# skhu101/HumanLiff

Measured on AMD Instinct MI355X. Metric: denoise-steps/sec, higher is better.
Workload: dtype f32; 1 GPU; configs[1]: 256x256x27 tri-plane UNet (controlnet, 497M params), 1000-step DDPM p_sample_loop, batch=4 per GPU; global_batch=4, parallelism=replicas x1 (subjects sharded, final all-gather only)

## Files before the change

humanliff_amd/csrc/hl_unet.cpp:

```cpp
#include <cstdint>
#include <string>
#include <unordered_map>
#include <utility>
#include <vector>

#include "hl_unet_kernels.h"
#include <algorithm>

namespace {

using hl::ConvArgs;
using hl::View;

static inline int round_up(int v, int m) { return (v + m - 1) / m * m; }

bool conv_mode_known(int mode) {
    return mode == HL_CONV_FP32 || mode == HL_CONV_FP32_MFMA || mode == HL_CONV_BF16X3 || mode == HL_CONV_FP32_DIRECT || mode == HL_CONV_FP32_F23 ||
           mode == HL_CONV_BF16 || mode == HL_CONV_FP16;
}
struct ConvForms { bool bf3, wino, wino4, h2, h16; };
ConvForms conv_forms(int mode, bool bf16_h16, bool bwd_data) {
    const bool f32 = mode == HL_CONV_FP32 || mode == HL_CONV_FP32_MFMA || mode == HL_CONV_FP16;
    ConvForms f;
    f.bf3 = mode == HL_CONV_BF16X3 || mode == HL_CONV_BF16;
    f.wino = f32 || mode == HL_CONV_FP32_F23;
    f.wino4 = f32;
    f.h2 = mode == HL_CONV_FP32 && !bwd_data;
    f.h16 = mode == HL_CONV_FP16 || (bf16_h16 && mode == HL_CONV_BF16);
    return f;
}

struct Conv {
    const float *w = nullptr;
    const void *w_bf3 = nullptr;
    const float *w_wino = nullptr;
    const void *w_h2 = nullptr;
    const void *w_h16 = nullptr;
    const float *w_wino4 = nullptr;
    const float *bias = nullptr;
    int Cin = 0, Cin_pad = 0, Cout = 0, ks = 1;
};
struct Norm {
    const float *gamma = nullptr, *beta = nullptr;
    int C = 0;
    float eps = 1e-5f;
};
struct Res {
    Norm n1, n2;
    Conv c1, c2, skip;
    bool has_skip = false;
    bool aware = false;
    long emb_off = 0;
    int Cin = 0, Cout = 0;
};
struct Attn {
    Norm norm;
    Conv qkv, proj;
    int C = 0, heads = 1;
};
struct Xf {
    Norm norm;
    Conv proj_in, proj_out, qkv, out1, ff_in, ff_out;
    const float *ln1_g = nullptr, *ln1_b = nullptr, *ln3_g = nullptr, *ln3_b = nullptr;
    const float *v2_w = nullptr, *o2_w = nullptr, *o2_b = nullptr;
    int C = 0, heads = 1;
};
enum Kind { K_CONV, K_RES, K_ATTN, K_DOWN, K_UP, K_XF };
struct Layer {
    Kind kind;
    int idx;
};
struct Block {
    std::vector<Layer> layers;
    int Cout = 0;
    int ds_out = 1;
};

struct Net {
    hl_unet_cfg cfg{};
    std::unordered_map<std::string, std::pair<const float *, int64_t>> sd;
    std::vector<Conv> convs;
    std::vector<Res> res;
    std::vector<Attn> attn;
    std::vector<Xf> xf;
    std::vector<Block> in_blocks, out_blocks, cond_blocks;
    Block middle;
    std::vector<int> proj_cond;
    Conv out_conv;
    Norm out_norm;
    const float *te0_w = nullptr, *te0_b = nullptr, *te2_w = nullptr, *te2_b = nullptr, *label = nullptr;
    Conv ada1, ada2;
    const float *ada_w = nullptr, *ada_b = nullptr;
    const float *emb_w = nullptr, *emb_b = nullptr;
    long emb_total = 0;
    int E = 0;
    int Cpad0 = 0;
    float *packed = nullptr;
    size_t packed_off = 0;
    bool dry = true;
    hipStream_t st = nullptr;
    std::string err;
    hipStream_t side = nullptr;
    hipEvent_t ev_fork = nullptr, ev_join = nullptr;
    std::vector<hipEvent_t> ev_block;
    bool overlap = true;
    int conv_mode = 0;
    bool prof = false;
    std::vector<hipEvent_t> ev_pool;
    struct Span { int cat; size_t a, b; double flops, exec; int key[5]; long mid; };
    double dom[4] = {0, 0, 0, 0};
    int dom_key[5] = {0, 0, 0, 0, 0};
    std::vector<Span> spans;
    size_t ev_used = 0;
    int64_t census[5][8] = {};
    ~Net() {
        for (auto e : ev_pool) if (e) hipEventDestroy(e);
        for (auto e : ev_block) if (e) hipEventDestroy(e);
        if (ev_fork) hipEventDestroy(ev_fork);
        if (ev_join) hipEventDestroy(ev_join);
        if (side) hipStreamDestroy(side);
    }
    size_t next_event() {
        if (ev_used == ev_pool.size()) {
            hipEvent_t e = nullptr;
            if (hipEventCreate(&e) != hipSuccess) { if (err.empty()) err = "hipEventCreate failed (profiling events)"; e = nullptr; }
            ev_pool.push_back(e);
        }
        return ev_used++;
    }
};
enum { CAT_CONV = 0, CAT_GN = 1, CAT_ATTN = 2, CAT_OTHER = 3, CAT_N = 4 };

const float *lookup(Net &n, const std::string &name, int64_t expect) {
    if (n.dry) return reinterpret_cast<const float *>(16);
    auto it = n.sd.find(name);
    if (it == n.sd.end()) { if (n.err.empty()) n.err = "missing state_dict key: " + name; return nullptr; }
    if (expect >= 0 && it->second.second != expect) {
        if (n.err.empty()) n.err = "shape mismatch for " + name + ": got " + std::to_string(it->second.second) + " elements, expected " + std::to_string(expect);
        return nullptr;
    }
    return it->second.first;
}

Conv make_conv_w(Net &n, const float *w, const float *bias, int Cin, int Cout, int ks);
Conv make_conv(Net &n, const std::string &p, int Cin, int Cout, int ks, bool has_bias = true) {
    const float *w = lookup(n, p + ".weight", (int64_t)Cout * Cin * ks * ks);
    const float *b = has_bias ? lookup(n, p + ".bias", Cout) : nullptr;
    return make_conv_w(n, w, b, Cin, Cout, ks);
}
Conv make_conv_w(Net &n, const float *w, const float *bias, int Cin, int Cout, int ks) {
    Conv c;
    c.Cin = Cin; c.Cin_pad = round_up(Cin, 16); c.Cout = Cout; c.ks = ks;
    c.bias = n.dry ? nullptr : bias;
    const int cp = c.Cin_pad;
    size_t wino4 = hl::conv_packed_wino4_bytes(Cout, cp, ks);
    if (wino4 > ((size_t)64 << 20)) wino4 = 0;
    const size_t bytes[6] = {hl::conv_packed_floats(Cout, cp, ks) * sizeof(float), hl::conv_packed_bf3_bytes(Cout, cp, ks),
                             hl::conv_packed_wino_bytes(Cout, cp, ks), wino4, hl::conv_packed_h2_bytes(Cout, cp, ks),
                             hl::conv_packed_h16_bytes(Cout, cp, ks)};
    for (int f = 0; f < 6; ++f) {
        if (!bytes[f]) continue;
        float *dst = n.dry ? nullptr : n.packed + n.packed_off;
        n.packed_off += (bytes[f] / 4 + 63) / 64 * 64;
        if (n.dry || !w) continue;
        int rc = 0;
        switch (f) {
        case 0: rc = hl::conv_pack_weights(w, Cout, Cin, cp, ks, dst, n.st); c.w = dst; break;
        case 1: rc = hl::conv_pack_weights_bf3(w, Cout, Cin, cp, ks, dst, n.st); c.w_bf3 = dst; break;
        case 2: rc = hl::conv_pack_weights_wino(w, Cout, Cin, cp, dst, n.st); c.w_wino = dst; break;
        case 3: rc = hl::conv_pack_weights_wino4(w, Cout, Cin, cp, dst, n.st); c.w_wino4 = dst; break;
        case 4: rc = hl::conv_pack_weights_h2(w, Cout, Cin, cp, ks, dst, n.st); c.w_h2 = dst; break;
        default: rc = hl::conv_pack_weights_h16(w, Cout, Cin, cp, ks, dst, 1, n.st); c.w_h16 = dst; break;
        }
        if (rc != 0 && n.err.empty()) n.err = hl_last_error();
    }
    return c;
}
Norm make_norm(Net &n, const std::string &p, int C) {
    Norm g;
    g.C = C;
    g.gamma = lookup(n, p + ".weight", C);
    g.beta = lookup(n, p + ".bias", C);
    return g;
}

struct EmbPiece { std::string name; int O; long off; };

int add_res(Net &n, std::vector<EmbPiece> &emb, const std::string &p, int Cin, int Cout, bool aware = false) {
    Res r;
    r.Cin = Cin; r.Cout = Cout; r.aware = aware;
    r.n1 = make_norm(n, p + ".in_layers.0", Cin);
    r.c1 = make_conv(n, p + ".in_layers.2", Cin, Cout, 3);
    r.emb_off = n.emb_total;
    const int emb_o = n.cfg.no_scale_shift ? Cout : 2 * Cout;
    emb.push_back({p + ".emb_layers.1", emb_o, n.emb_total});
    n.emb_total += emb_o;
    r.n2 = make_norm(n, p + ".out_layers.0", Cout);
    r.c2 = make_conv(n, p + ".out_layers.3", aware ? 3 * Cout : Cout, Cout, 3);
    r.has_skip = Cin != Cout;
    if (r.has_skip) {
        int ks = 1;
        if (!n.dry) {
            auto it = n.sd.find(p + ".skip_connection.weight");
            if (it != n.sd.end() && it->second.second == (int64_t)Cout * Cin * 9) ks = 3;
        }
        r.skip = make_conv(n, p + ".skip_connection", Cin, Cout, ks);
        if (n.dry) n.packed_off += hl::conv_packed_floats(Cout, round_up(Cin, 16), 3) * 5;
    }
    n.res.push_back(r);
    return (int)n.res.size() - 1;
}
int add_attn(Net &n, const std::string &p, int C, int heads) {
    Attn a;
    a.C = C; a.heads = heads;
    a.norm = make_norm(n, p + ".norm", C);
    a.qkv = make_conv(n, p + ".qkv", C, 3 * C, 1);
    a.proj = make_conv(n, p + ".proj_out", C, C, 1);
    n.attn.push_back(a);
    return (int)n.attn.size() - 1;
}
int add_xf(Net &n, const std::string &p, int C, int heads) {
    Xf a;
    a.C = C; a.heads = heads;
    a.norm = make_norm(n, p + ".norm", C);
    a.norm.eps = 1e-6f;
    a.proj_in = make_conv(n, p + ".proj_in", C, C, 1);
    const std::string t = p + ".transformer_blocks.0";
    const int d = C / heads;
    const float *wq = lookup(n, t + ".attn1.to_q.weight", (int64_t)C * C), *wk = lookup(n, t + ".attn1.to_k.weight", (int64_t)C * C),
                *wv = lookup(n, t + ".attn1.to_v.weight", (int64_t)C * C);
    float *fused = n.dry ? nullptr : n.packed + n.packed_off;
    n.packed_off += ((size_t)3 * C * C + 63) / 64 * 64;
    if (!n.dry && wq && wk && wv) {
        const float *src[3] = {wq, wk, wv};
        for (int h = 0; h < heads; ++h)
            for (int q = 0; q < 3; ++q)
                hipMemcpyAsync(fused + ((size_t)h * 3 + q) * d * C, src[q] + (size_t)h * d * C, (size_t)d * C * sizeof(float), hipMemcpyDeviceToDevice, n.st);
    }
    a.qkv = make_conv_w(n, n.dry ? reinterpret_cast<const float *>(16) : fused, nullptr, C, 3 * C, 1);
    a.out1 = make_conv(n, t + ".attn1.to_out.0", C, C, 1);
    a.ln1_g = lookup(n, t + ".norm1.weight", C); a.ln1_b = lookup(n, t + ".norm1.bias", C);
    a.ln3_g = lookup(n, t + ".norm3.weight", C); a.ln3_b = lookup(n, t + ".norm3.bias", C);
    a.v2_w = lookup(n, t + ".attn2.to_v.weight", (int64_t)C * n.E);
    a.o2_w = lookup(n, t + ".attn2.to_out.0.weight", (int64_t)C * C);
    a.o2_b = lookup(n, t + ".attn2.to_out.0.bias", C);
    a.ff_in = make_conv(n, t + ".ff.net.0.proj", C, 8 * C, 1);
    a.ff_out = make_conv(n, t + ".ff.net.2", 4 * C, C, 1);
    a.proj_out = make_conv(n, p + ".proj_out", C, C, 1);
    n.xf.push_back(a);
    return (int)n.xf.size() - 1;
}
int add_conv(Net &n, const std::string &p, int Cin, int Cout, int ks) {
    n.convs.push_back(make_conv(n, p, Cin, Cout, ks));
    return (int)n.convs.size() - 1;
}
bool has_ds(const hl_unet_cfg &c, int ds) {
    for (int i = 0; i < c.n_attention_ds; ++i)
        if (c.attention_ds[i] == ds) return true;
    return false;
}

void build_encoder(Net &n, std::vector<EmbPiece> &emb, const std::string &root, std::vector<Block> &blocks,
                   std::vector<int> &chans, bool aware) {
    const hl_unet_cfg &c = n.cfg;
    Block b0;
    b0.layers.push_back({K_CONV, add_conv(n, root + ".0.0", c.in_channels, c.model_channels, 3)});
    b0.Cout = c.model_channels;
    b0.ds_out = 1;
    blocks.push_back(b0);
    chans.push_back(c.model_channels);
    int ch = c.model_channels, ds = 1, bi = 1;
    for (int level = 0; level < c.n_levels; ++level) {
        for (int r = 0; r < c.num_res_blocks; ++r) {
            Block b;
            const std::string p = root + "." + std::to_string(bi);
            const int co = c.channel_mult[level] * c.model_channels;
            b.layers.push_back({K_RES, add_res(n, emb, p + ".0", ch, co, aware)});
            ch = co;
            if (has_ds(c, ds)) {
                if (c.cross_attn) b.layers.push_back({K_XF, add_xf(n, p + ".1", ch, c.num_heads)});
                else b.layers.push_back({K_ATTN, add_attn(n, p + ".1", ch, c.num_heads)});
            }
            b.Cout = ch; b.ds_out = ds;
            blocks.push_back(b);
            chans.push_back(ch);
            ++bi;
        }
        if (level != c.n_levels - 1) {
            Block b;
            const std::string p = root + "." + std::to_string(bi);
            b.layers.push_back({K_DOWN, add_conv(n, p + ".0.op", ch, ch, 3)});
            ds *= 2;
            b.Cout = ch; b.ds_out = ds;
            blocks.push_back(b);
            chans.push_back(ch);
            ++bi;
        }
    }
}

void build(Net &n) {
    const hl_unet_cfg &c = n.cfg;
    n.E = 4 * c.model_channels;
    n.Cpad0 = round_up(c.in_channels, 16);
    n.emb_total = 0;
    n.packed_off = 0;
    n.convs.clear(); n.res.clear(); n.attn.clear(); n.xf.clear();
    n.in_blocks.clear(); n.out_blocks.clear(); n.cond_blocks.clear(); n.proj_cond.clear();
    std::vector<EmbPiece> emb;
    n.te0_w = lookup(n, "time_embed.0.weight", (int64_t)n.E * c.model_channels);
    n.te0_b = lookup(n, "time_embed.0.bias", n.E);
    n.te2_w = lookup(n, "time_embed.2.weight", (int64_t)n.E * n.E);
    n.te2_b = lookup(n, "time_embed.2.bias", n.E);
    n.label = c.num_classes > 0 ? lookup(n, "label_emb.weight", (int64_t)c.num_classes * n.E) : nullptr;
    if (c.adagn || c.cross_attn) {
        n.ada1 = make_conv(n, "conv_proj_1", c.out_channels, 6, 3);
        n.ada2 = make_conv(n, "conv_proj_2", 6, 1, 3);
        n.ada_w = lookup(n, "linear.weight", (int64_t)n.E * 4096);
        n.ada_b = lookup(n, "linear.bias", n.E);
    }

    std::vector<int> chans;
    const bool aware = c.aware3d != 0;
    build_encoder(n, emb, "input_blocks", n.in_blocks, chans, aware);
    int ch = chans.back();
    int ds = n.in_blocks.back().ds_out;
    {
        Block m;
        m.layers.push_back({K_RES, add_res(n, emb, "middle_block.0", ch, ch, aware)});
        if (c.cross_attn) m.layers.push_back({K_XF, add_xf(n, "middle_block.1", ch, c.num_heads)});
        else m.layers.push_back({K_ATTN, add_attn(n, "middle_block.1", ch, c.num_heads)});
        m.layers.push_back({K_RES, add_res(n, emb, "middle_block.2", ch, ch, aware)});
        m.Cout = ch; m.ds_out = ds;
        n.middle = m;
    }
    std::vector<int> stack = chans;
    int bi = 0;
    for (int level = c.n_levels - 1; level >= 0; --level) {
        for (int i = 0; i <= c.num_res_blocks; ++i) {
            Block b;
            const std::string p = "output_blocks." + std::to_string(bi);
            const int skip = stack.back();
            stack.pop_back();
            const int co = c.model_channels * c.channel_mult[level];
            int li = 0;
            b.layers.push_back({K_RES, add_res(n, emb, p + "." + std::to_string(li++), ch + skip, co, aware)});
            ch = co;
            if (has_ds(c, ds)) {
                if (c.cross_attn) b.layers.push_back({K_XF, add_xf(n, p + "." + std::to_string(li++), ch, c.num_heads)});
                else b.layers.push_back({K_ATTN, add_attn(n, p + "." + std::to_string(li++), ch, c.num_heads_upsample)});
            }
            if (level && i == c.num_res_blocks) {
                b.layers.push_back({K_UP, add_conv(n, p + "." + std::to_string(li++) + ".conv", ch, ch, 3)});
                ds /= 2;
            }
            b.Cout = ch; b.ds_out = ds;
            n.out_blocks.push_back(b);
            ++bi;
        }
    }
    n.out_norm = make_norm(n, "out.0", ch);
    n.out_conv = make_conv(n, "out.2", c.model_channels, c.out_channels, 3);
    if (c.controlnet) {
        std::vector<int> cch;
        build_encoder(n, emb, "input_blocks_cond", n.cond_blocks, cch, false);
        for (size_t i = 0; i < n.cond_blocks.size(); ++i)
            n.proj_cond.push_back(add_conv(n, "input_blocks_proj_cond." + std::to_string(i), cch[i], cch[i], 1));
    }
    const size_t wfl = (size_t)n.emb_total * n.E;
    if (!n.dry) {
        float *wdst = n.packed + n.packed_off, *bdst = wdst + wfl;
        for (auto &e : emb) {
            const float *w = lookup(n, e.name + ".weight", (int64_t)e.O * n.E);
            const float *b = lookup(n, e.name + ".bias", e.O);
            if (!w || !b) continue;
            hipMemcpyAsync(wdst + (size_t)e.off * n.E, w, (size_t)e.O * n.E * sizeof(float), hipMemcpyDeviceToDevice, n.st);
            hipMemcpyAsync(bdst + e.off, b, (size_t)e.O * sizeof(float), hipMemcpyDeviceToDevice, n.st);
        }
        n.emb_w = wdst; n.emb_b = bdst;
    }
    n.packed_off += (wfl + n.emb_total + 63) / 64 * 64;
}

struct Exec {
    Net &n;
    bool run;
    char *ws;
    size_t off = 0;
    hipStream_t st;
    int B, H, W;
    float *emb_all = nullptr;
    const float *ctx = nullptr;
    float *gn_scratch = nullptr;
    float *splitk_ws = nullptr;
    float *gn_scratch2 = nullptr, *splitk_ws2 = nullptr;
    float *act_ws = nullptr, *act_ws2 = nullptr;
    size_t act_need = 0;
    int rc = 0;
    struct StatReg { float *buf; int viewC, c0, covered; };
    struct PartInfo { float *buf; int viewC, c0; };
    std::unordered_map<const float *, PartInfo> part_reg;
    char *stat_base = nullptr;
    size_t stat_off = 0, stat_bytes = 0;
    float *alloc_stat(size_t floats) {
        float *p = run ? reinterpret_cast<float *>(stat_base + stat_off) : nullptr;
        stat_off += (floats * sizeof(float) + 255) / 256 * 256;
        return p;
    }
    std::unordered_map<const float *, StatReg> stat_reg;
    bool want_stats = true;

    float *alloc(size_t floats) {
        float *p = run ? reinterpret_cast<float *>(ws + off) : nullptr;
        off += (floats * sizeof(float) + 255) / 256 * 256;
        return p;
    }
    View plain(int ds, int C) {
        View v;
        v.N = B; v.H = H / ds; v.W = W / ds; v.C = C; v.pitch = C;
        v.p = alloc((size_t)v.pixels() * C);
        return v;
    }
    void ok(int r) { if (r && !rc) rc = r; }
    size_t span_begin() {
        if (!n.prof) return 0;
        const size_t a = n.next_event();
        if (n.ev_pool[a]) hipEventRecord(n.ev_pool[a], st);
        return a;
    }
    void span_end(int cat, size_t a, double flops, double exec = -1.0) {
        if (!n.prof) return;
        if (!n.err.empty() && !rc) rc = hl::fail(HL_ERR_RUNTIME, "hl_unet_forward: %s", n.err.c_str());
        const size_t b = n.next_event();
        if (n.ev_pool[b]) hipEventRecord(n.ev_pool[b], st);
        n.spans.push_back({cat, a, b, flops, exec < 0 ? flops : exec, {span_key[0], span_key[1], span_key[2], span_key[3], span_key[4]}, span_mid});
        span_key[0] = -1; span_mid = -1;
    }
    int span_key[5] = {-1, 0, 0, 0, 0};
    long span_mid = -1;

    struct Aff { float *cA = nullptr, *cB = nullptr; hl::GnSrc gn{}; bool on = false; };
    const Aff none{};
    void conv(const Conv &c, const View &in, const View &out, int stride, int ups, const Aff &af, int act,
              const float *res, long res_pitch, float *out2 = nullptr, long out2_pitch = 0, const float *res2 = nullptr,
              long res2_pitch = 0, int nchw = 0) {
        const float *cA = af.cA, *cB = af.cB;
        if (!run) {
            const size_t need = (size_t)in.pixels() * c.Cin_pad;
            if (need > act_need) act_need = need;
        }
        const bool st_ok = want_stats && !nchw;
        PartInfo pi1{nullptr, c.Cout, 0}, pi2{nullptr, c.Cout, 0};
        if (st_ok) {
            auto f1 = run ? part_reg.find(out.p) : part_reg.end();
            if (f1 != part_reg.end()) pi1 = f1->second; else pi1.buf = alloc_stat(hl::conv_stats_floats(B, (long)out.H * out.W));
            if (out2_pitch != 0) {
                auto f2 = run ? part_reg.find(out2) : part_reg.end();
                if (f2 != part_reg.end()) pi2 = f2->second; else pi2.buf = alloc_stat(hl::conv_stats_floats(B, (long)out.H * out.W));
            }
        }
        float *st1 = pi1.buf, *st2 = pi2.buf;
        if (!run) return;
        ConvArgs a{};
        a.in = in; a.in.C = c.Cin_pad;
        const ConvForms f = conv_forms(n.conv_mode, false, false);
        a.w = c.w; a.w_bf3 = f.bf3 ? c.w_bf3 : nullptr; a.bf16_single = n.conv_mode == HL_CONV_BF16;
        a.w_wino = f.wino ? c.w_wino : nullptr; a.w_wino4 = f.wino4 ? c.w_wino4 : nullptr;
        a.w_h16 = f.h16 ? c.w_h16 : nullptr; a.h16_fp16 = 1;
        a.w_h2 = f.h2 ? c.w_h2 : nullptr;
        a.bias = c.bias; a.Cout = c.Cout; a.ks = c.ks; a.stride = stride; a.ups = ups;
        a.coefA = cA; a.coefB = cB; a.act = act; a.gn = af.gn;
        a.out = out; a.res = res; a.res_pitch = res_pitch;
        a.out2 = out2; a.out2_pitch = out2_pitch; a.res2 = res2; a.res2_pitch = res2_pitch; a.out_nchw = nchw;
        a.splitk_ws = splitk_ws; a.splitk_ws_bytes = hl::conv_splitk_ws_bytes();
        a.act_ws = act_ws; a.act_ws_bytes = act_need * sizeof(float);
        a.stats = st1; a.stats2 = st2;
        if (af.cA == nullptr && af.gn.gt == nullptr) a.in_stats = raw_totals(in);
        a.st_cg = pi1.viewC / 32; a.st_c0 = pi1.c0; a.st2_cg = pi2.viewC / 32; a.st2_c0 = pi2.c0;
        const size_t e0 = span_begin();
        size_t emid = 0;
        if (n.prof) { emid = n.next_event(); a.ev_mid = n.ev_pool[emid]; }
        const hl::ConvPlan pl = hl::plan_conv(a);
        ok(hl::conv2d(a, pl, st));
        {
            static const int audit_ = [] { const char *e_ = getenv("HL_AUDIT_SCALE"); return e_ ? atoi(e_) : 0; }();
            if (audit_ && pl.path == hl::ConvPath::Fp16x2 && af.cA == nullptr && af.gn.gt == nullptr && a.in_stats == nullptr)
                fprintf(stderr, "[hl audit] fp16x2 convolution with an unscaled raw input: %dx%d px, %d -> %d channels, ks %d, stride %d\n", in.H, in.W, in.C, c.Cout, c.ks, stride);
        }
        if (n.prof && a.ev_mid && pl.pre != hl::ConvPrePass::None) span_mid = (long)emid;
        {
            int lvl = 0;
            while (lvl < 7 && (out.H << lvl) < H) ++lvl;
            n.census[hl::conv_census_row(pl.path)][lvl] += 1;
            span_key[0] = (int)pl.path; span_key[1] = lvl; span_key[2] = ups ? 1 : 0; span_key[3] = c.Cout; span_key[4] = c.ks;
        }
        const double fl = 2.0 * (double)out.pixels() * c.Cout * c.Cin * c.ks * c.ks;
        span_end(CAT_CONV, e0, fl, fl * hl::conv_issued_factor(pl.path));
        if (pl.stat_slots > 0) {
            stat_reg[out.p] = {st1, pi1.viewC, pi1.c0, c.Cout};
            if (out2) stat_reg[out2] = {st2, pi2.viewC, pi2.c0, c.Cout};
        } else {
            stat_reg.erase(out.p);
            if (out2) stat_reg.erase(out2);
        }
    }
    const float *raw_totals(const View &x) const {
        auto it = stat_reg.find(x.p);
        if (it == stat_reg.end() || it->second.c0 != 0) return nullptr;
        if (it->second.covered == x.C) return it->second.buf;
        auto it2 = stat_reg.find(x.p + it->second.covered);
        if (it2 != stat_reg.end() && it2->second.buf == it->second.buf && it2->second.c0 == it->second.covered &&
            it->second.covered + it2->second.covered == x.C) return it->second.buf;
        return nullptr;
    }
    Aff coef(const View &x, const Norm &g, const float *emb, bool force_arrays = false) {
        Aff af;
        af.on = true;
        af.cA = alloc((size_t)B * x.C);
        af.cB = alloc((size_t)B * x.C);
        if (!run) return af;
        const float *gt = nullptr;
        auto it = stat_reg.find(x.p);
        if (it != stat_reg.end() && it->second.viewC == x.C && it->second.c0 == 0) {
            if (it->second.covered == x.C) gt = it->second.buf;
            else {
                auto it2 = stat_reg.find(x.p + it->second.covered);
                if (it2 != stat_reg.end() && it2->second.buf == it->second.buf && it2->second.c0 == it->second.covered &&
                    it->second.covered + it2->second.covered == x.C) gt = it->second.buf;
            }
        }
        if (gt && !force_arrays && !n.prof) {
            af.cA = af.cB = nullptr;
            af.gn.gt = gt; af.gn.C = x.C; af.gn.HW = x.H * x.W;
            af.gn.gamma = g.gamma; af.gn.beta = g.beta; af.gn.emb = emb; af.gn.emb_pitch = n.emb_total; af.gn.eps = g.eps;
            return af;
        }
        const size_t e0 = span_begin();
        if (gt) ok(hl::groupnorm_coef_stats(x, gt, g.gamma, g.beta, emb, n.emb_total, af.cA, af.cB, st, g.eps));
        else ok(hl::groupnorm_coef(x, g.gamma, g.beta, emb, n.emb_total, af.cA, af.cB, gn_scratch, st, nullptr, g.eps));
        span_end(CAT_GN, e0, 0.0);
        return af;
    }
    void res_block(const Res &r, const View &x, const View &dst) {
        Aff a1 = coef(x, r.n1, nullptr), a2;
        View h = plain(H / dst.H, r.Cout);
        if (n.cfg.no_scale_shift) {
            want_stats = false;
            conv(r.c1, x, h, 1, 0, a1, 1, nullptr, 0);
            want_stats = true;
            if (run) ok(hl::add_rowvec(h, emb_all + r.emb_off, st, n.emb_total));
            a2 = coef(h, r.n2, nullptr, r.aware);
        } else {
            conv(r.c1, x, h, 1, 0, a1, 1, nullptr, 0);
            a2 = coef(h, r.n2, run ? emb_all + r.emb_off : nullptr, r.aware);
        }
        if (r.aware) {
            View h3 = plain(H / dst.H, 3 * r.Cout);
            float *sums = alloc((size_t)B * 3 * (h.H + h.W / 3) * r.Cout);
            if (run) {
                const size_t e0 = span_begin();
                ok(hl::gn_apply_3d(h, a2.cA, a2.cB, sums, h3.p, st));
                span_end(CAT_GN, e0, 0.0);
            }
            if (r.has_skip) {
                want_stats = false;
                conv(r.skip, x, dst, 1, 0, none, 0, nullptr, 0);
                want_stats = true;
                conv(r.c2, h3, dst, 1, 0, none, 0, dst.p, dst.pitch);
            } else {
                conv(r.c2, h3, dst, 1, 0, none, 0, x.p, x.pitch);
            }
            return;
        }
        if (r.has_skip) {
            want_stats = false;
            conv(r.skip, x, dst, 1, 0, none, 0, nullptr, 0);
            want_stats = true;
            conv(r.c2, h, dst, 1, 0, a2, 1, dst.p, dst.pitch);
        } else {
            conv(r.c2, h, dst, 1, 0, a2, 1, x.p, x.pitch);
        }
    }
    void attn_block(const Attn &a, const View &x, const View &dst) {
        const Aff af = coef(x, a.norm, nullptr);
        View qkv = plain(H / x.H, 3 * a.C);
        want_stats = false;
        conv(a.qkv, x, qkv, 1, 0, af, 0, nullptr, 0);
        want_stats = true;
        View o = plain(H / x.H, a.C);
        float *ost = alloc_stat(hl::conv_stats_floats(B, (long)x.H * x.W));
        if (run) {
            const size_t e0 = span_begin();
            int emitted = 0;
            ok(hl::attention(qkv.p, B, x.H * x.W, a.C, a.heads, o.p, st, n.conv_mode == HL_CONV_FP32, ost, &emitted));
            if (emitted) stat_reg[o.p] = {ost, a.C, 0, a.C}; else stat_reg.erase(o.p);
            const double T = (double)x.H * x.W;
            span_end(CAT_ATTN, e0, 4.0 * B * T * T * a.C);
        }
        conv(a.proj, o, dst, 1, 0, none, 0, x.p, x.pitch);
    }
    void xf_block(const Xf &a, const View &x, const View &dst) {
        const int ds = H / x.H;
        const Aff af = coef(x, a.norm, nullptr);
        const bool ws_keep = want_stats;
        want_stats = false;
        View h = plain(ds, a.C), ln = plain(ds, a.C), qkv = plain(ds, 3 * a.C), o = plain(ds, a.C), h1 = plain(ds, a.C);
        View ln3 = plain(ds, a.C), f8 = plain(ds, 8 * a.C), f4 = plain(ds, 4 * a.C), h2 = plain(ds, a.C);
        float *v2 = alloc((size_t)B * a.C), *r2 = alloc((size_t)B * a.C);
        conv(a.proj_in, x, h, 1, 0, af, 0, nullptr, 0);
        if (run) ok(hl::layernorm(h, a.ln1_g, a.ln1_b, ln.p, st));
        conv(a.qkv, ln, qkv, 1, 0, none, 0, nullptr, 0);
        if (run) {
            const size_t e0 = span_begin();
            ok(hl::attention(qkv.p, B, x.H * x.W, a.C, a.heads, o.p, st, n.conv_mode == HL_CONV_FP32));
            const double T = (double)x.H * x.W;
            span_end(CAT_ATTN, e0, 4.0 * B * T * T * a.C);
        }
        conv(a.out1, o, h1, 1, 0, none, 0, h.p, h.pitch);
        if (run) {
            ok(hl::linear_small(ctx, n.E, B, n.E, a.v2_w, nullptr, a.C, 0, nullptr, nullptr, v2, a.C, st));
            ok(hl::linear_small(v2, a.C, B, a.C, a.o2_w, a.o2_b, a.C, 0, nullptr, nullptr, r2, a.C, st));
            ok(hl::add_rowvec(h1, r2, st));
            ok(hl::layernorm(h1, a.ln3_g, a.ln3_b, ln3.p, st));
        }
        conv(a.ff_in, ln3, f8, 1, 0, none, 0, nullptr, 0);
        if (run) ok(hl::geglu(f8.p, f8.pixels(), 4 * a.C, f4.p, st));
        conv(a.ff_out, f4, h2, 1, 0, none, 0, h1.p, h1.pitch);
        want_stats = ws_keep;
        conv(a.proj_out, h2, dst, 1, 0, none, 0, x.p, x.pitch);
    }
    void block(const Block &b, View x, const View &dst) {
        for (size_t i = 0; i < b.layers.size(); ++i) {
            const Layer &L = b.layers[i];
            const bool last = i + 1 == b.layers.size();
            int Cout, ds_out;
            const int ds_in = H / x.H;
            switch (L.kind) {
                case K_CONV: Cout = n.convs[L.idx].Cout; ds_out = ds_in; break;
                case K_RES: Cout = n.res[L.idx].Cout; ds_out = ds_in; break;
                case K_ATTN: Cout = n.attn[L.idx].C; ds_out = ds_in; break;
                case K_XF: Cout = n.xf[L.idx].C; ds_out = ds_in; break;
                case K_DOWN: Cout = n.convs[L.idx].Cout; ds_out = ds_in * 2; break;
                default: Cout = n.convs[L.idx].Cout; ds_out = ds_in / 2; break;
            }
            View y = last ? dst : plain(ds_out, Cout);
            switch (L.kind) {
                case K_CONV: conv(n.convs[L.idx], x, y, 1, 0, none, 0, nullptr, 0); break;
                case K_RES: res_block(n.res[L.idx], x, y); break;
                case K_ATTN: attn_block(n.attn[L.idx], x, y); break;
                case K_XF: xf_block(n.xf[L.idx], x, y); break;
                case K_DOWN: conv(n.convs[L.idx], x, y, 2, 0, none, 0, nullptr, 0); break;
                case K_UP: conv(n.convs[L.idx], x, y, 1, 1, none, 0, nullptr, 0); break;
            }
            x = y;
        }
    }

    void forward(const float *x, const int64_t *t, const float *tf, const float *x_cond, const int64_t *y, float *out) {
        const hl_unet_cfg &c = n.cfg;
        if (run && stat_bytes) ok(hipMemsetAsync(stat_base, 0, stat_bytes, st) == hipSuccess ? 0 : hl::fail(HL_ERR_RUNTIME, "hl_unet_forward: memset of the statistics arena"));
        gn_scratch = alloc(hl::gn_scratch_floats(B));
        splitk_ws = alloc(hl::conv_splitk_ws_bytes() / sizeof(float));
        gn_scratch2 = alloc(hl::gn_scratch_floats(B));
        splitk_ws2 = alloc(hl::conv_splitk_ws_bytes() / sizeof(float));
        float *temb = alloc((size_t)B * c.model_channels), *e1 = alloc((size_t)B * n.E), *emb = alloc((size_t)B * n.E);
        emb_all = alloc((size_t)B * n.emb_total);
        View xin; xin.N = B; xin.H = H; xin.W = W; xin.C = n.Cpad0; xin.pitch = n.Cpad0;
        xin.p = alloc((size_t)xin.pixels() * n.Cpad0);
        View xsum = xin;
        if (c.controlnet) xsum.p = alloc((size_t)xin.pixels() * n.Cpad0);
        float *xin_tot = alloc_stat(hl::conv_stats_floats(B, (long)H * W)), *xsum_tot = alloc_stat(hl::conv_stats_floats(B, (long)H * W));
        View ac, a1, a2;
        float *emb0 = nullptr;
        int64_t *iota = nullptr;
        if (c.adagn || c.cross_attn) {
            ac.N = B; ac.H = H; ac.W = W; ac.C = round_up(c.out_channels, 16); ac.pitch = ac.C; ac.p = alloc((size_t)ac.pixels() * ac.C);
            a1.N = B; a1.H = H / 2; a1.W = W / 2; a1.C = 16; a1.pitch = 16; a1.p = alloc((size_t)a1.pixels() * 16);
            a2.N = B; a2.H = H / 4; a2.W = W / 4; a2.C = 1; a2.pitch = 1; a2.p = alloc((size_t)a2.pixels());
            emb0 = alloc((size_t)B * n.E);
            iota = reinterpret_cast<int64_t *>(alloc(2 * 16));
            if (run) {
                static const int64_t h_iota[16] = {0, 1, 2, 3, 4, 5, 6, 7, 8, 9, 10, 11, 12, 13, 14, 15};
                ok(hipMemcpyAsync(iota, h_iota, sizeof(h_iota), hipMemcpyHostToDevice, st) == hipSuccess ? 0 : hl::fail(HL_ERR_RUNTIME, "hl_unet_forward: memcpy"));
                ok(hipMemsetAsync(a1.p, 0, (size_t)a1.pixels() * 16 * sizeof(float), st) == hipSuccess ? 0 : hl::fail(HL_ERR_RUNTIME, "hl_unet_forward: memset"));
                ok(hl::prep_inputs(x_cond, nullptr, B, c.out_channels, H, W, ac.C, ac.p, nullptr, st));
            }
            View a1w = a1; a1w.C = 6;
            conv(n.ada1, ac, a1w, 2, 0, none, 0, nullptr, 0);
            conv(n.ada2, a1, a2, 2, 0, none, 0, nullptr, 0);
        }
        if (run) {
            const size_t e0 = span_begin();
            ok(hl::timestep_embedding(t, tf, B, c.model_channels, temb, st));
            ok(hl::linear_small(temb, c.model_channels, B, c.model_channels, n.te0_w, n.te0_b, n.E, 0, nullptr, nullptr, e1, n.E, st));
            ok(hl::linear_small(e1, n.E, B, n.E, n.te2_w, n.te2_b, n.E, 1, c.num_classes > 0 ? n.label : nullptr, y, c.adagn ? emb0 : emb, n.E, st));
            ctx = emb0;
            if (c.adagn) ok(hl::linear_small(a2.p, 4096, B, 4096, n.ada_w, n.ada_b, n.E, 0, emb0, iota, emb, n.E, st));
            if (c.cross_attn) ok(hl::linear_small(a2.p, 4096, B, 4096, n.ada_w, n.ada_b, n.E, 0, nullptr, nullptr, emb0, n.E, st));
            ok(hl::linear_small(emb, n.E, B, n.E, n.emb_w, n.emb_b, (int)n.emb_total, 1, nullptr, nullptr, emb_all, n.emb_total, st));
            if (c.aware3d) ok(hl::prep_inputs_3d(x, c.controlnet ? x_cond : nullptr, B, c.in_channels, H, W / 3, n.Cpad0, xin.p,
                                                 c.controlnet ? xsum.p : nullptr, st));
            else {
                ok(hl::prep_inputs(x, c.controlnet ? x_cond : nullptr, B, c.in_channels, H, W, n.Cpad0, xin.p,
                                   c.controlnet ? xsum.p : nullptr, st, xin_tot, c.controlnet ? xsum_tot : nullptr));
                stat_reg[xin.p] = {xin_tot, n.Cpad0, 0, n.Cpad0};
                if (c.controlnet) stat_reg[xsum.p] = {xsum_tot, n.Cpad0, 0, n.Cpad0};
            }
            span_end(CAT_OTHER, e0, 2.0 * B * ((double)n.E * c.model_channels + (double)n.E * n.E + (double)n.emb_total * n.E));
        }
        const size_t nb = n.in_blocks.size();
        std::vector<View> cat(nb);
        {
            int ch = n.middle.Cout;
            for (size_t j = 0; j < nb; ++j) {
                const Block &src = n.in_blocks[nb - 1 - j];
                cat[j] = plain(src.ds_out, ch + src.Cout);
                ch = n.out_blocks[j].Cout;
            }
        }
        {
            std::vector<float *> cat_st(nb);
            for (size_t j = 0; j < nb; ++j) cat_st[j] = alloc_stat(hl::conv_stats_floats(B, (long)cat[j].H * cat[j].W));
            if (run && c.controlnet) {
                int ch = n.middle.Cout;
                for (size_t j = 0; j < nb; ++j) {
                    part_reg[cat[j].p] = {cat_st[j], cat[j].C, 0};
                    part_reg[cat[j].p + ch] = {cat_st[j], cat[j].C, ch};
                    ch = n.out_blocks[j].Cout;
                }
            }
        }
        auto first_part = [&](size_t j, int C) { View v = cat[j]; v.C = C; return v; };
        const bool fork = run && c.controlnet && n.overlap && !n.prof && n.side;
        hipStream_t main_st = st;
        if (fork) {
            hipEventRecord(n.ev_fork, main_st);
            hipStreamWaitEvent(n.side, n.ev_fork, 0);
        }
        std::vector<View> hs(nb);
        View h = xin;
        for (size_t i = 0; i < nb; ++i) {
            hs[i] = plain(n.in_blocks[i].ds_out, n.in_blocks[i].Cout);
            block(n.in_blocks[i], h, hs[i]);
            if (fork) hipEventRecord(n.ev_block[i], main_st);
            h = hs[i];
        }
        block(n.middle, h, first_part(0, n.middle.Cout));
        if (c.controlnet) {
            if (fork) { st = n.side; std::swap(gn_scratch, gn_scratch2); std::swap(splitk_ws, splitk_ws2); std::swap(act_ws, act_ws2); }
            View hc = xsum;
            for (size_t i = 0; i < nb; ++i) {
                View tmp = plain(n.cond_blocks[i].ds_out, n.cond_blocks[i].Cout);
                block(n.cond_blocks[i], hc, tmp);
                View pj = plain(n.cond_blocks[i].ds_out, n.cond_blocks[i].Cout);
                const size_t j = nb - 1 - i;
                const int Ch = cat[j].C - hs[i].C;
                if (fork) hipStreamWaitEvent(n.side, n.ev_block[i], 0);
                conv(n.convs[n.proj_cond[i]], tmp, pj, 1, 0, none, 0, nullptr, 0,
                     run ? cat[j].p + Ch : nullptr, cat[j].pitch, hs[i].p, hs[i].pitch);
                hc = pj;
            }
            if (fork) {
                hipEventRecord(n.ev_join, n.side);
                st = main_st; std::swap(gn_scratch, gn_scratch2); std::swap(splitk_ws, splitk_ws2); std::swap(act_ws, act_ws2);
                hipStreamWaitEvent(main_st, n.ev_join, 0);
            }
        } else if (run) {
            for (size_t i = 0; i < nb; ++i) {
                const size_t j = nb - 1 - i;
                const int Ch = cat[j].C - hs[i].C;
                hipMemcpy2DAsync(cat[j].p + Ch, cat[j].pitch * sizeof(float), hs[i].p, hs[i].pitch * sizeof(float),
                                 (size_t)hs[i].C * sizeof(float), (size_t)hs[i].pixels(), hipMemcpyDeviceToDevice, st);
                stat_reg.erase(cat[j].p + Ch);
            }
        }
        View last;
        for (size_t j = 0; j < nb; ++j) {
            View dst = (j + 1 < nb) ? first_part(j + 1, n.out_blocks[j].Cout) : plain(n.out_blocks[j].ds_out, n.out_blocks[j].Cout);
            block(n.out_blocks[j], cat[j], dst);
            last = dst;
        }
        const Aff afo = coef(last, n.out_norm, nullptr);
        View o; o.N = B; o.H = H; o.W = W; o.C = c.out_channels; o.pitch = c.out_channels; o.p = out;
        if (c.aware3d) {
            o.p = alloc((size_t)o.pixels() * c.out_channels);
            conv(n.out_conv, last, o, 1, 0, afo, 1, nullptr, 0, nullptr, 0, nullptr, 0, 1);
            if (run) ok(hl::unroll_planes(o.p, B, c.out_channels, H, W / 3, out, st));
            return;
        }
        conv(n.out_conv, last, o, 1, 0, afo, 1, nullptr, 0, nullptr, 0, nullptr, 0, 1);
    }
};

int validate(const hl_unet_cfg *c) {
    HL_REQUIRE(c, "unet: null cfg");
    HL_REQUIRE(c->n_levels >= 1 && c->n_levels <= 8 && c->n_attention_ds >= 0 && c->n_attention_ds <= 8, "unet: bad cfg sizes");
    HL_REQUIRE(c->model_channels % 32 == 0, "unet: model_channels must be a multiple of 32 (GroupNorm32)");
    HL_REQUIRE(c->in_channels > 0 && c->out_channels > 0 && c->num_res_blocks > 0 && c->num_heads > 0, "unet: bad cfg");
    HL_REQUIRE(!(c->controlnet && c->adagn), "unet: cond_type is either controlnet or AdaGN");
    HL_REQUIRE(!(c->aware3d && (c->adagn || c->cross_attn)), "unet: use_3d_aware with cond_type='AdaGN' / 'cross_attention' is not built");
    HL_REQUIRE(c->controlnet + c->adagn + c->cross_attn <= 1, "unet: one cond_type");
    return 0;
}

}

extern "C" {

size_t hl_unet_packed_bytes(const hl_unet_cfg *cfg) {
    if (validate(cfg)) return 0;
    Net n;
    n.cfg = *cfg;
    if (n.cfg.num_heads_upsample <= 0) n.cfg.num_heads_upsample = n.cfg.num_heads;
    n.dry = true;
    build(n);
    return n.packed_off * sizeof(float) + 256;
}

int hl_unet_create(const hl_unet_cfg *cfg, int n_tensors, const char *const *names, const void *const *ptrs,
                   const int64_t *numels, void *packed, void *stream, void **handle) {
    int rc = validate(cfg);
    if (rc) return rc;
    HL_REQUIRE(names && ptrs && numels && packed && handle, "hl_unet_create: null argument");
    Net *n = new Net();
    n->cfg = *cfg;
    if (n->cfg.num_heads_upsample <= 0) n->cfg.num_heads_upsample = n->cfg.num_heads;
    for (int i = 0; i < n_tensors; ++i) n->sd[names[i]] = {static_cast<const float *>(ptrs[i]), numels[i]};
    n->dry = false;
    n->packed = static_cast<float *>(packed);
    n->st = (hipStream_t)stream;
    build(*n);
    if (!n->err.empty()) {
        rc = hl::fail(HL_ERR_INVALID, "hl_unet_create: %s", n->err.c_str());
        delete n;
        return rc;
    }
    if (n->cfg.controlnet) {
        bool okc = hipStreamCreateWithFlags(&n->side, hipStreamNonBlocking) == hipSuccess;
        okc = okc && hipEventCreateWithFlags(&n->ev_fork, hipEventDisableTiming) == hipSuccess;
        okc = okc && hipEventCreateWithFlags(&n->ev_join, hipEventDisableTiming) == hipSuccess;
        n->ev_block.assign(n->in_blocks.size(), nullptr);
        for (auto &e : n->ev_block) okc = okc && hipEventCreateWithFlags(&e, hipEventDisableTiming) == hipSuccess;
        if (!okc) {
            (void)hipGetLastError();
            if (n->side) { hipStreamDestroy(n->side); n->side = nullptr; }
        }
    }
    *handle = n;
    return HL_OK;
}

int hl_unet_set_overlap(void *handle, int enable) {
    HL_REQUIRE(handle, "hl_unet_set_overlap: null handle");
    static_cast<Net *>(handle)->overlap = enable != 0;
    return HL_OK;
}

int hl_unet_set_conv_mode(void *handle, int mode) {
    HL_REQUIRE(handle, "hl_unet_set_conv_mode: null handle");
    HL_REQUIRE(conv_mode_known(mode), "hl_unet_set_conv_mode: unknown mode %d", mode);
    static_cast<Net *>(handle)->conv_mode = mode;
    return HL_OK;
}

void hl_unet_destroy(void *handle) { delete static_cast<Net *>(handle); }

size_t hl_unet_workspace_bytes(void *handle, int B, int H, int W) {
    if (!handle || B <= 0) return 0;
    Net &n = *static_cast<Net *>(handle);
    Exec e{n, false, nullptr, 0, nullptr, B, H, n.cfg.aware3d ? 3 * W : W};
    e.forward(nullptr, nullptr, nullptr, nullptr, nullptr, nullptr);
    return e.off + 2 * e.act_need * sizeof(float) + e.stat_off + 1024;
}

int hl_unet_forward(void *handle, const float *x, const int64_t *t, const float *t_float, const float *x_cond,
                    const int64_t *y, float *out, int B, int H, int W, void *workspace, void *stream) {
    HL_REQUIRE(handle && x && (t || t_float) && out && workspace, "hl_unet_forward: null argument");
    Net &n = *static_cast<Net *>(handle);
    const int total_ds = 1 << (n.cfg.n_levels - 1);
    HL_REQUIRE(B >= 1 && B <= 16, "hl_unet_forward: batch %d outside [1,16]", B);
    HL_REQUIRE(H % total_ds == 0 && W % total_ds == 0, "hl_unet_forward: H,W must be divisible by %d", total_ds);
    HL_REQUIRE(!n.cfg.controlnet || x_cond, "hl_unet_forward: x_cond is required with cond_type='controlnet'");
    HL_REQUIRE(!(n.cfg.adagn || n.cfg.cross_attn) || (x_cond && H == 256 && W == 256),
               "hl_unet_forward: cond_type='AdaGN' / 'cross_attention' need x_cond and 256x256 inputs (Linear(64*64, ..))");
    HL_REQUIRE(n.cfg.num_classes == 0 || y, "hl_unet_forward: y is required for a class-conditional model");
    if (n.cfg.aware3d) W *= 3;
    Exec dry{n, false, nullptr, 0, nullptr, B, H, W};
    dry.forward(nullptr, nullptr, nullptr, nullptr, nullptr, nullptr);
    Exec e{n, true, static_cast<char *>(workspace), 0, (hipStream_t)stream, B, H, W};
    e.act_need = dry.act_need;
    e.act_ws = reinterpret_cast<float *>(static_cast<char *>(workspace) + (dry.off + 255) / 256 * 256);
    e.act_ws2 = e.act_ws + dry.act_need;
    e.stat_base = reinterpret_cast<char *>(e.act_ws2 + dry.act_need);
    e.stat_base += (256 - (reinterpret_cast<uintptr_t>(e.stat_base) & 255)) & 255;
    e.stat_bytes = dry.stat_off;
    for (auto &row : n.census) for (auto &v : row) v = 0;
    e.forward(x, t, t_float, x_cond, y, out);
    return e.rc;
}

int hl_unet_dispatch_census(void *handle, int64_t *h_counts) {
    HL_REQUIRE(handle && h_counts, "hl_unet_dispatch_census: null argument");
    const Net &n = *static_cast<Net *>(handle);
    for (int p = 0; p < 4; ++p) for (int l = 0; l < 8; ++l) h_counts[p * 8 + l] = n.census[p][l];
    return HL_OK;
}

int hl_unet_dispatch_census_ex(void *handle, int64_t *h_counts, int rows) {
    HL_REQUIRE(handle && h_counts && rows >= 1 && rows <= 5, "hl_unet_dispatch_census_ex: bad argument");
    const Net &n = *static_cast<Net *>(handle);
    for (int p = 0; p < rows; ++p) for (int l = 0; l < 8; ++l) h_counts[p * 8 + l] = n.census[p][l];
    return HL_OK;
}

int hl_unet_profile(void *handle, int enable) {
    HL_REQUIRE(handle, "hl_unet_profile: null handle");
    Net &n = *static_cast<Net *>(handle);
    n.prof = enable != 0;
    n.spans.clear();
    n.ev_used = 0;
    return HL_OK;
}

int hl_unet_profile_read(void *handle, double *h_ms, double *h_flops, int64_t *h_launches) {
    return hl_unet_profile_read_ex(handle, h_ms, h_flops, nullptr, h_launches);
}

int hl_unet_profile_read_ex(void *handle, double *h_ms, double *h_flops, double *h_exec_flops, int64_t *h_launches) {
    HL_REQUIRE(handle && h_ms && h_flops && h_launches, "hl_unet_profile_read: null argument");
    Net &n = *static_cast<Net *>(handle);
    for (int i = 0; i < CAT_N; ++i) { h_ms[i] = 0; h_flops[i] = 0; h_launches[i] = 0; if (h_exec_flops) h_exec_flops[i] = 0; }
    if (n.spans.empty()) return HL_OK;
    HL_HIP(hipEventSynchronize(n.ev_pool[n.spans.back().b]));
    struct Agg { double ms = 0, fl = 0, ex = 0; long calls = 0; int key[5]; };
    std::vector<Agg> aggs;
    for (auto &sp : n.spans) {
        float ms = 0.f;
        HL_HIP(hipEventElapsedTime(&ms, n.ev_pool[sp.a], n.ev_pool[sp.b]));
        h_ms[sp.cat] += ms; h_flops[sp.cat] += sp.flops; h_launches[sp.cat] += 1;
        if (h_exec_flops) h_exec_flops[sp.cat] += sp.exec;
        if (sp.cat == CAT_CONV && sp.key[0] >= 0) {
            Agg *hit = nullptr;
            for (auto &g : aggs) if (std::equal(g.key, g.key + 5, sp.key)) { hit = &g; break; }
            if (!hit) { aggs.emplace_back(); hit = &aggs.back(); std::copy(sp.key, sp.key + 5, hit->key); }
            float kms = ms;
            if (sp.mid >= 0 && n.ev_pool[sp.mid]) HL_HIP(hipEventElapsedTime(&kms, n.ev_pool[sp.mid], n.ev_pool[sp.b]));
            hit->ms += kms; hit->fl += sp.flops; hit->ex += sp.exec; hit->calls += 1;
        }
    }
    n.dom[0] = n.dom[1] = n.dom[2] = n.dom[3] = 0;
    for (auto &g : aggs)
        if (g.ms > n.dom[0]) {
            n.dom[0] = g.ms; n.dom[1] = g.fl / g.calls; n.dom[2] = g.ex / g.calls; n.dom[3] = (double)g.calls;
            std::copy(g.key, g.key + 5, n.dom_key);
        }
    n.spans.clear();
    n.ev_used = 0;
    return HL_OK;
}

int hl_unet_profile_dominant(void *handle, double *h_vals, int *h_key) {
    HL_REQUIRE(handle && h_vals && h_key, "hl_unet_profile_dominant: null argument");
    const Net &n = *static_cast<Net *>(handle);
    for (int i = 0; i < 4; ++i) h_vals[i] = n.dom[i];
    for (int i = 0; i < 5; ++i) h_key[i] = n.dom_key[i];
    return HL_OK;
}

static int g_single_op_scale_from_totals = 0;
static int conv2d_single(int mode, const float *in, int N, int H, int W, int Cin, const float *w_oihw, const float *bias, int Cout,
                         int ks, int stride, int upsample, const float *coefA, const float *coefB, int silu,
                         const float *residual, float *out, void *scratch, size_t scratch_bytes, void *stream,
                         float *stats = nullptr, int *stat_slots = nullptr, int tf = 0, int Cin_w = -1, long out_pitch = 0) {
    HL_REQUIRE(Cin % 16 == 0, "hl_conv2d_nhwc: Cin must be a multiple of 16");
    if (Cin_w < 0) Cin_w = Cin;
    HL_REQUIRE(Cin_w <= Cin, "hl_conv2d_nhwc: the weight has more input channels than the tensor");
    hipStream_t st = (hipStream_t)stream;
    const size_t need32 = (hl::conv_packed_floats(Cout, Cin, ks) * sizeof(float) + 255) / 256 * 256;
    const ConvForms f = conv_forms(mode, true, tf != 0);
    const size_t b_bf3 = f.bf3 ? hl::conv_packed_bf3_bytes(Cout, Cin, ks) : 0, b_wino = f.wino ? hl::conv_packed_wino_bytes(Cout, Cin, ks) : 0,
                 b_wino4 = f.wino4 ? hl::conv_packed_wino4_bytes(Cout, Cin, ks) : 0, b_h2 = f.h2 ? hl::conv_packed_h2_bytes(Cout, Cin, ks) : 0,
                 b_h16 = f.h16 ? hl::conv_packed_h16_bytes(Cout, Cin, ks) : 0;
    const size_t extra = std::max({b_bf3, b_wino, b_wino4, b_h2, b_h16});
    const size_t need = need32 + (extra + 255) / 256 * 256;
    HL_REQUIRE(scratch && scratch_bytes >= need, "hl_conv2d_nhwc: scratch too small (%zu < %zu)", scratch_bytes, need);
    ConvArgs a{};
    void *extra_dst = static_cast<char *>(scratch) + need32;
    a.in.p = const_cast<float *>(in); a.in.N = N; a.in.H = H; a.in.W = W; a.in.C = Cin; a.in.pitch = Cin;
    a.w = static_cast<float *>(scratch); a.bias = bias; a.Cout = Cout; a.ks = ks; a.stride = stride; a.ups = upsample;
    if (b_bf3) { a.w_bf3 = extra_dst; a.bf16_single = mode == HL_CONV_BF16; }
    if (b_wino) a.w_wino = static_cast<float *>(extra_dst);
    if (b_wino4) a.w_wino4 = static_cast<float *>(extra_dst);
    if (b_h16) { a.w_h16 = extra_dst; a.h16_fp16 = mode == HL_CONV_FP16; }
    if (b_h2) a.w_h2 = extra_dst;
    a.coefA = coefA; a.coefB = coefB; a.act = silu;
// ... 157 lines not shown
```

Baseline: 152.3 denoise-steps/s.

## Overlap residual-block skip 1x1 convs on side stream with main path

Runs the skip-connection conv of residual blocks that have one on a secondary stream, forking at block entry and joining before the second conv that accumulates into the same destination. The side stream is used only once the controlnet fork has joined (or when there is no controlnet), with scratch buffers swapped so the two streams do not collide. This is meant to hide the small skip conv behind the GroupNorm and first conv of the main path. The cost is extra event record/wait overhead per block and possible contention for compute units.

```diff
diff --git a/humanliff_amd/csrc/hl_unet.cpp b/humanliff_amd/csrc/hl_unet.cpp
--- a/humanliff_amd/csrc/hl_unet.cpp
+++ b/humanliff_amd/csrc/hl_unet.cpp
@@ -103,6 +103,7 @@
     hipStream_t side = nullptr;
     hipEvent_t ev_fork = nullptr, ev_join = nullptr;
     std::vector<hipEvent_t> ev_block;
+    std::vector<hipEvent_t> ev_skip;
     bool overlap = true;
     int conv_mode = 0;
     bool prof = false;
@@ -116,6 +117,7 @@
     ~Net() {
         for (auto e : ev_pool) if (e) hipEventDestroy(e);
         for (auto e : ev_block) if (e) hipEventDestroy(e);
+        for (auto e : ev_skip) if (e) hipEventDestroy(e);
         if (ev_fork) hipEventDestroy(ev_fork);
         if (ev_join) hipEventDestroy(ev_join);
         if (side) hipStreamDestroy(side);
@@ -409,6 +411,8 @@
     }
     std::unordered_map<const float *, StatReg> stat_reg;
     bool want_stats = true;
+    bool side_free = false;
+    void swap_scratch() { std::swap(gn_scratch, gn_scratch2); std::swap(splitk_ws, splitk_ws2); std::swap(act_ws, act_ws2); }
 
     float *alloc(size_t floats) {
         float *p = run ? reinterpret_cast<float *>(ws + off) : nullptr;
@@ -541,7 +545,25 @@
         span_end(CAT_GN, e0, 0.0);
         return af;
     }
+    void skip_conv(const Res &r, const View &x, const View &dst, bool on_side) {
+        const size_t i = (size_t)(&r - n.res.data());
+        hipStream_t main_st = st;
+        if (on_side) {
+            hipStreamWaitEvent(n.side, n.ev_skip[2 * i], 0);
+            st = n.side; swap_scratch();
+        }
+        want_stats = false;
+        conv(r.skip, x, dst, 1, 0, none, 0, nullptr, 0);
+        want_stats = true;
+        if (on_side) {
+            hipEventRecord(n.ev_skip[2 * i + 1], n.side);
+            st = main_st; swap_scratch();
+            hipStreamWaitEvent(main_st, n.ev_skip[2 * i + 1], 0);
+        }
+    }
     void res_block(const Res &r, const View &x, const View &dst) {
+        const bool on_side = run && side_free && r.has_skip;
+        if (on_side) hipEventRecord(n.ev_skip[2 * (size_t)(&r - n.res.data())], st);
         Aff a1 = coef(x, r.n1, nullptr), a2;
         View h = plain(H / dst.H, r.Cout);
         if (n.cfg.no_scale_shift) {
@@ -563,9 +585,7 @@
                 span_end(CAT_GN, e0, 0.0);
             }
             if (r.has_skip) {
-                want_stats = false;
-                conv(r.skip, x, dst, 1, 0, none, 0, nullptr, 0);
-                want_stats = true;
+                skip_conv(r, x, dst, on_side);
                 conv(r.c2, h3, dst, 1, 0, none, 0, dst.p, dst.pitch);
             } else {
                 conv(r.c2, h3, dst, 1, 0, none, 0, x.p, x.pitch);
@@ -573,9 +593,7 @@
             return;
         }
         if (r.has_skip) {
-            want_stats = false;
-            conv(r.skip, x, dst, 1, 0, none, 0, nullptr, 0);
-            want_stats = true;
+            skip_conv(r, x, dst, on_side);
             conv(r.c2, h, dst, 1, 0, a2, 1, dst.p, dst.pitch);
         } else {
             conv(r.c2, h, dst, 1, 0, a2, 1, x.p, x.pitch);
@@ -731,7 +749,9 @@
             }
         }
         auto first_part = [&](size_t j, int C) { View v = cat[j]; v.C = C; return v; };
-        const bool fork = run && c.controlnet && n.overlap && !n.prof && n.side;
+        const bool two_streams = run && n.overlap && !n.prof && n.side;
+        const bool fork = two_streams && c.controlnet;
+        side_free = two_streams && !fork;
         hipStream_t main_st = st;
         if (fork) {
             hipEventRecord(n.ev_fork, main_st);
@@ -747,7 +767,7 @@
         }
         block(n.middle, h, first_part(0, n.middle.Cout));
         if (c.controlnet) {
-            if (fork) { st = n.side; std::swap(gn_scratch, gn_scratch2); std::swap(splitk_ws, splitk_ws2); std::swap(act_ws, act_ws2); }
+            if (fork) { st = n.side; swap_scratch(); }
             View hc = xsum;
             for (size_t i = 0; i < nb; ++i) {
                 View tmp = plain(n.cond_blocks[i].ds_out, n.cond_blocks[i].Cout);
@@ -762,8 +782,9 @@
             }
             if (fork) {
                 hipEventRecord(n.ev_join, n.side);
-                st = main_st; std::swap(gn_scratch, gn_scratch2); std::swap(splitk_ws, splitk_ws2); std::swap(act_ws, act_ws2);
+                st = main_st; swap_scratch();
                 hipStreamWaitEvent(main_st, n.ev_join, 0);
+                side_free = true;
             }
         } else if (run) {
             for (size_t i = 0; i < nb; ++i) {
@@ -835,12 +856,15 @@
         delete n;
         return rc;
     }
-    if (n->cfg.controlnet) {
+    {
         bool okc = hipStreamCreateWithFlags(&n->side, hipStreamNonBlocking) == hipSuccess;
         okc = okc && hipEventCreateWithFlags(&n->ev_fork, hipEventDisableTiming) == hipSuccess;
         okc = okc && hipEventCreateWithFlags(&n->ev_join, hipEventDisableTiming) == hipSuccess;
         n->ev_block.assign(n->in_blocks.size(), nullptr);
         for (auto &e : n->ev_block) okc = okc && hipEventCreateWithFlags(&e, hipEventDisableTiming) == hipSuccess;
+        n->ev_skip.assign(2 * n->res.size(), nullptr);
+        for (size_t i = 0; i < n->ev_skip.size(); ++i)
+            if (n->res[i / 2].has_skip) okc = okc && hipEventCreateWithFlags(&n->ev_skip[i], hipEventDisableTiming) == hipSuccess;
         if (!okc) {
             (void)hipGetLastError();
             if (n->side) { hipStreamDestroy(n->side); n->side = nullptr; }
```

Result: no change. 152.9 denoise-steps/s, median of 6 (+0.4%).
